# killerwhile/kafka-assignment-optimizer

Hardware: AMD Instinct MI355X
Metric: candidate assignments/sec (+ time_to_optimal_s), 10k-partition reassign (higher is better)
Workload: dtype int32

## Files before the change

### kafka_assignment_optimizer_amd/csrc/kao_search.hip

```cpp
#include "kao_search_dev.h"

namespace kao {

template <bool kGlobalA, bool kPriced, int NW, bool kWide, bool kTeam, bool kCurG = false, int RFT = 0>
__device__ __forceinline__ void search_body(unsigned char *smem, const SearchPools &pl, const SearchParams &prm) {
    static_assert(!kTeam || kGlobalA, "teams run topics that live in global memory");
    static_assert(!kCurG || !kGlobalA, "kCurG: the working assignment is in LDS");
    static_assert(RFT == 0 || (RFT == 3 && NW == 4 && !kGlobalA && !kTeam), "RFT = 3: LDS-resident topics of four words per partition");
    constexpr int NS = RFT ? RFT : NW;
    const int lane = threadIdx.x & 63;
    const int wave = __builtin_amdgcn_readfirstlane(threadIdx.x >> 6);
    const int n_waves = kTeam ? __builtin_amdgcn_readfirstlane((int)(blockDim.x >> 6)) : 1;
    const int tid = kTeam ? (int)threadIdx.x : lane, nthr = kTeam ? (int)blockDim.x : 64;
    const int2 bm = pl.block_map[blockIdx.x];
    const TopicDev *TD = pl.topics + bm.x;

    TopicRegs T = topic_regs<RFT>(TD);
    asm volatile("" : "+v"(T.rep_lo), "+v"(T.rep_hi), "+v"(T.lead_lo), "+v"(T.lead_hi));

    const int a_bytes = kGlobalA ? 0 : prm.maxP * NW * 4;
    const int cur_bytes = (kGlobalA || kCurG) ? 0 : prm.maxP * NW * 4;
    const int bx64 = (prm.maxBx + 63) & ~63;
    const int c_bytes = bx64 * 4;
    const int krt = search_rack_tab(prm.maxR);
// ... 164 lines not shown
    const uint32_t pmask = (1u << plog) - 1u;
    const uint32_t lrange = (uint32_t)(prm.lam_max - prm.lam_min + 1);
    const uint32_t RF8 = (uint32_t)T.RF << 8, R8 = (uint32_t)T.R << 8, m8 = (uint32_t)T.m << 8;

    const int T_tour = min(64, max(4, (T.P * T.RF) >> 2));
    uint32_t tour_off = lane < T_tour ? 0u : kKeyNull;
    asm volatile("" : "+v"(tour_off));
    const int GA = min(16, max(1, (T.P * T.RF) >> 8));
    const int x_rounds_full = (T.P + 63) >> 6;
    const bool x_windowed = x_rounds_full > 8;

    int lam_lo = prm.lam_min, lam_hi = prm.lam_max;
    uint32_t n_iters = prm.iters, it_base = prm.launch * prm.iters;
    uint32_t scan_two = TD->P * TD->RF <= prm.scan2_max ? 1u : 0u;
    {
        uint32_t v0 = (uint32_t)lam_lo, v1 = (uint32_t)lam_hi, v2 = n_iters, v3 = it_base, v4 = scan_two;
        asm volatile("" : "+v"(v0), "+v"(v1), "+v"(v2), "+v"(v3), "+v"(v4));
        lam_lo = (int)__builtin_amdgcn_readfirstlane(v0); lam_hi = (int)__builtin_amdgcn_readfirstlane(v1);
        n_iters = __builtin_amdgcn_readfirstlane(v2); it_base = __builtin_amdgcn_readfirstlane(v3);
        scan_two = __builtin_amdgcn_readfirstlane(v4);
    }
    constexpr bool kFuse = !kGlobalA && !kTeam && !kPriced;
    const bool fuse_ok = kFuse && T.Bx <= 16384;
    uint32_t jmp_a = 1u, jmp_c = 0u;
    if (fuse_ok)
        for (int n = (T.Bx + 63) >> 6; n > 0; --n) { jmp_a = (jmp_a * 0x6D2B79u) & 0xFFFFFFu; jmp_c = (jmp_c * 0x6D2B79u + 0x3C6EF3u) & 0xFFFFFFu; }
    for (uint32_t i = 0; i < n_iters; ++i) {
        const uint32_t it = it_base + i;
        const int type = (int)((0x1210u >> ((it & 7u) * 2u)) & 3u);
        const uint32_t ph = it & pmask;
        const int lam = best_obj < 0 ? lam_hi : min(lam_hi, lam_lo + (int)((2u * ph * lrange) >> plog));
        const bool sampled = (type == 2) || (type == 0 && ((it >> 3) & 1u));

        uint32_t key = kKeyNull;
        int dV = 0, dObj = 0, p = 0, k = 0, q = 0, j = 0;
        uint32_t uw = 0, vw = 0;
        uint32_t kmin;
        int win;

        if (sampled) {
            p = (int)rnd24_wide(rng, (uint32_t)T.P);
            const Part<NW> a = L.A[p];
            const Part<NW> c = CUR[p];
            if (type == 0) {
                k = (int)rnd24(rng, RF8);
                uw = sel_slot<NS>(a, k);
                const uint32_t ro = uw >> 16;
                const bool lead = k == 0;
                const uint32_t lw = lead ? 2u : 0u;
                const int wl = lead ? T.w00 : T.w01, wf = lead ? T.w10 : T.w11;
                const int g_old = role_w2<NS>(c, uw, wl, wf) + (hbw ? bw_of(BW[uw & 0xFFFFu], lead) : 0);
                const uint32_t wo = L.W[uw & 0xFFFFu];
                const int dV_old = wfld(wo, kWDecR) + wfldw(wo, kWDecL, lw);
                const int dV_rack_old = ddec(L.K[ro], T.rack_lo, T.rack_hi) + ddec(cnt4<NS>(a, ro), T.prack_lo, T.prack_hi);
                const int rsz_ro = RSZ[ro];
                int dP_old = 0, dP_rack_old = 0;
                if (kPriced) {
                    const uint32_t pro = PR[uw & 0xFFFFu];
                    dP_old = -(wflag(wo, kWPoutR) & price_rep(pro));
                    if (lead) dP_old -= wflag(wo, kWPoutL) & price_lead(pro);
                    dP_rack_old = p_out(L.K[ro], T.rack_lo, T.rack_hi, PG[ro]);
                }
#pragma unroll
                for (int g = 0; g < 4; ++g) {
                    uint32_t r, jj;
                    bool okg;
                    if (g < 2) {
                        r = rnd24(rng, R8);
                        jj = rnd24(rng, m8);
                        okg = (int)jj < RSZ[r];
                    } else {
                        r = ro;
                        jj = rnd24(rng, (uint32_t)rsz_ro << 8);
                        okg = true;
                    }
                    const uint32_t x = __umul24(r, (uint32_t)T.m) + jj;
                    const uint32_t xw = x | (r << 16);
                    okg = okg && !in4<NS>(a, xw);
                    const uint32_t wn = L.W[x];
                    int dVg = dV_old + wfld(wn, kWIncR) + wfldw(wn, kWIncL, lw);
                    if (g < 2) {
                        if (r != ro)
                            dVg += dV_rack_old + dinc(L.K[r], T.rack_lo, T.rack_hi) + dinc(cnt4<NS>(a, r), T.prack_lo, T.prack_hi);
                    }
                    const int dObjg = role_w2<NS>(c, xw, wl, wf) + (hbw ? bw_of(BW[x], lead) : 0) - g_old;
                    uint32_t keyg;
                    if (kPriced) {
                        const uint32_t prx = PR[x];
                        int dPg = dP_old + (wflag(wn, kWPinR) & price_rep(prx));
                        if (lead) dPg += wflag(wn, kWPinL) & price_lead(prx);
                        if (g < 2 && r != ro) dPg += dP_rack_old + p_in(L.K[r], T.rack_lo, T.rack_hi, PG[r]);
                        keyg = okg ? make_key_p(lam, S, dVg, dObjg, dPg, lane) : kKeyNull;
                    }
                    else keyg = okg ? make_key(lam, S, dVg, dObjg, lane) : kKeyNull;
                    if (keyg < key) { key = keyg; vw = xw; dV = dVg; dObj = dObjg; }
                }
            } else {
                uw = a.w[0];
                const int u_lead = role_w2<NS>(c, uw, T.w00, T.w10), u_fol = role_w2<NS>(c, uw, T.w01, T.w11);
                const uint32_t wu = L.W[uw & 0xFFFFu];
                const int dV_u = wfld(wu, kWDecL);
                const int dP_u = kPriced ? -(wflag(wu, kWPoutL) & price_lead(PR[uw & 0xFFFFu])) : 0;
#pragma unroll
                for (int kk = 1; kk < NS; ++kk) {
                    if (!RFT && kk >= T.RF) break;
                    const uint32_t xw = a.w[kk];
                    const int dObjg = role_w2<NS>(c, xw, T.w00, T.w10) + u_fol - u_lead - role_w2<NS>(c, xw, T.w01, T.w11) +
                                      (hbw ? (int)(BW[xw & 0xFFFFu] >> 16) - (int)(BW[uw & 0xFFFFu] >> 16) : 0);
                    const uint32_t wx = L.W[xw & 0xFFFFu];
                    const int dVg = dV_u + wfld(wx, kWIncL);
                    uint32_t keyg;
                    if (kPriced) keyg = make_key_p(lam, S, dVg, dObjg, dP_u + (wflag(wx, kWPinL) & price_lead(PR[xw & 0xFFFFu])), lane);
                    else keyg = make_key(lam, S, dVg, dObjg, lane);
                    if (keyg < key) { key = keyg; vw = xw; k = kk; dV = dVg; dObj = dObjg; }
                }
            }
            kmin = wave_umin(key);
            win = (int)(kmin & 63u);
        } else {
            uint32_t keyA, oldw_l;
            int pl_, kl_, g_old_l, dvo_l = 0, dvr_l = 0;
            auto score_words = [&](auto ty, uint32_t &key_o, const Part<NW> &al, const Part<NW> &cl, int k_o, uint32_t &oldw_o, int &g_o, int &dvo_o, int &dvr_o) {
                constexpr int TY = decltype(ty)::value;
                oldw_o = sel_slot<NS>(al, k_o);
                const uint32_t rol = oldw_o >> 16;
                const bool leadl = k_o == 0;
                g_o = role_w2<NS>(cl, oldw_o, leadl ? T.w00 : T.w01, leadl ? T.w10 : T.w11);
                if (hbw && TY == 0) g_o += bw_of(BW[oldw_o & 0xFFFFu], leadl);
                const uint32_t wo = L.W[oldw_o & 0xFFFFu];
                const int dv7 = ddec(cnt4<NS>(al, rol), T.prack_lo, T.prack_hi);
                int sc;
                if (TY == 0) {
                    dvo_o = wfld(wo, kWDecR) + wfldw(wo, kWDecL, leadl ? 2u : 0u);
                    dvr_o = ddec(L.K[rol], T.rack_lo, T.rack_hi) + dv7;
                    sc = dvo_o + min(dvr_o, 0);
                } else {
                    const int dvl = wfld(wo, leadl ? kWDecL : kWIncL);
                    sc = min(dv7, 0) + min(dvl, 0);
                }
                if (kPriced) {
                    int dPs = 0;
                    if (TY == 0) {
                        const uint32_t pro = PR[oldw_o & 0xFFFFu];
                        dPs = -(wflag(wo, kWPoutR) & price_rep(pro));
                        dPs -= wflagw(wo, kWPoutL, leadl ? 1u : 0u) & price_lead(pro);
                    }
                    key_o = make_key_p(lam, S, sc, -g_o, dPs, lane) | tour_off;
                }
                else key_o = make_key(lam, S, sc, -g_o, lane) | tour_off;
            };
            auto score_slot = [&](auto ty, uint32_t &key_o, int p_o, int &k_o, uint32_t &oldw_o, int &g_o, int &dvo_o, int &dvr_o) {
// ... 133 lines not shown
                    int d2 = __mul24(lam, inc + wfldw(w, kWIncL, lw2) + (rt >> 16)) + K02;
                    if (decltype(with_w)::value) {
                        const uint32_t x = (uint32_t)(base + lane);
                        const uint32_t xw = x | ((uint32_t)XR[x] << 16);
                        d1 -= __mul24(S, role_w2<NS>(c1, xw, wl1, wf1));
                        d2 -= __mul24(S, role_w2<NS>(c2, xw, wl2, wf2));
                    }
                    d1 = min(max(d1, 0), 2 * kDBias - 2);
                    d2 = min(max(d2, 0), 2 * kDBias - 2) | wflag(w, 14);
                    key1 = ((uint32_t)d1 << 16) | (st1 & 0xFF00u) | (uint32_t)rd | ((uint32_t)w & 0xFFFF0000u);
                    key2 = ((uint32_t)d2 << 16) | (st2 & 0xFF00u) | (uint32_t)rd;
                };
                const int n_rd = (T.Bx + 63) >> 6;
                int rd = 0, base = 0;
                while (rd < n_rd) {
                    int nxt = n_rd;
#pragma unroll
                    for (int i2 = 0; i2 < 2 * NW; ++i2)
                        if (mr[i2] >= rd) nxt = min(nxt, mr[i2]);
                    uint32_t k1a, k2a, k1b, k2b;
                    for (; rd + 1 < nxt; rd += 2, base += 128) {
                        scan_round2(std::false_type{}, base, rd, k1a, k2a);
                        scan_round2(std::false_type{}, base + 64, rd + 1, k1b, k2b);
                        best1 = min(best1, min(k1a, k1b));
                        best2 = min(best2, min(k2a, k2b));
                    }
                    if (rd < nxt) { scan_round2(std::false_type{}, base, rd, k1a, k2a); best1 = min(best1, k1a); best2 = min(best2, k2a); ++rd; base += 64; }
                    if (rd < n_rd) { scan_round2(std::true_type{}, base, rd, k1a, k2a); best1 = min(best1, k1a); best2 = min(best2, k2a); ++rd; base += 64; }
                }
                asm("v_mad_u32_u24 %0, %0, %1, %2" : "+v"(rng) : "s"(jmp_a), "v"(jc));
                if (holds) L.W[ai & 0xFFFFu] = (uint16_t)w_keep;
                const uint32_t kw = wave_umin(min(((best1 >> 1) & ~127u) | (uint32_t)lane, ((best2 >> 1) & ~127u) | 64u | (uint32_t)lane));
                const bool two = (kw & 64u) != 0u;
                kmin = kw >> 7;
                win = (int)(kw & 63u);
                p = two ? ps[1] : ps[0]; k = two ? ks[1] : ks[0]; uw = two ? us[1] : us[0];
                if ((int)(kmin >> 8) - kDBias <= 0) {
                    const bool lead = k == 0;
                    const uint32_t bw_ = (uint32_t)__builtin_amdgcn_readlane((int)(two ? best2 : best1), win);
                    const uint32_t xs = ((bw_ & 255u) << 6) + (uint32_t)win;
                    const uint32_t rs = XR[xs];
                    const uint32_t ws = L.W[xs];
                    const int rts = L.RT[rs];
                    vw = xs | (rs << 16);
                    dV = wfld(ws, kWIncR) + wfldw(ws, kWIncL, lead ? 2u : 0u) + (two ? dvos[1] : dvos[0]) + (two ? (rts >> 16) : wfldw(rts, 0, 16u));
                    int mx1 = -1, mx2 = -1;
#pragma unroll
                    for (int i2 = 0; i2 < NW; ++i2) { mx1 = max(mx1, mr[i2]); mx2 = max(mx2, mr[NW + i2]); }
                    const bool has_missing = (two ? mx2 : mx1) >= 0;
                    dObj = -(two ? gs[1] : gs[0]) + (has_missing ? (two ? role_w2<NS>(c2, vw, wl2, wf2) : role_w2<NS>(c1, vw, wl1, wf1)) : 0);
                }
            } else {
            uint32_t b_kmin = kKeyNull, b_uw = 0, b_vw = 0;
            int b_win = 0, b_p = 0, b_k = 0, b_dV = 0, b_dObj = 0;
#pragma nounroll
            for (int si = 0; si < (wA2 >= 0 ? 2 : 1); ++si) {
            const int wA = si == 0 ? wA1 : wA2;
            p = __builtin_amdgcn_readlane(pl_, wA);
            k = __builtin_amdgcn_readlane(kl_, wA);
            uw = (uint32_t)__builtin_amdgcn_readlane((int)oldw_l, wA);
            const int g_old = __builtin_amdgcn_readlane(g_old_l, wA);
            const int dV_old = __builtin_amdgcn_readlane(dvo_l, wA);
            const int dV_rack_old = __builtin_amdgcn_readlane(dvr_l, wA);
            Part<NW> a, c;
            if constexpr (kGlobalA) {
#pragma unroll
                for (int i2 = 0; i2 < NW; ++i2) { a.w[i2] = (uint32_t)__builtin_amdgcn_readlane((int)a_l.w[i2], wA); c.w[i2] = (uint32_t)__builtin_amdgcn_readlane((int)c_l.w[i2], wA); }
            } else {
                a = L.A[p];
                c = CUR[p];
            }
            const bool lead = k == 0;
            const uint32_t ro = uw >> 16;
            if (type == 0) {
                {
                    const int dP_rack_old = kPriced ? p_out(L.K[ro], T.rack_lo, T.rack_hi, PG[ro]) : 0;
                    for (int r = lane; r < T.R; r += 64) {
                        int v = ((uint32_t)r != ro) ? dV_rack_old + dinc(L.K[r], T.rack_lo, T.rack_hi) + dinc(cnt4<NS>(a, (uint32_t)r), T.prack_lo, T.prack_hi) : 0;
                        if (kPriced)
                            v = (v & 0xFF) | ((((uint32_t)r != ro) ? dP_rack_old + p_in(L.K[r], T.rack_lo, T.rack_hi, PG[r]) : 0) * 256);
                        L.RT[r] = v;
                    }
                }
                const int wl = lead ? T.w00 : T.w01, wf = lead ? T.w10 : T.w11;
                const int li = lane & (NW - 1);
                const uint32_t ai = sel_slot<NS>(a, li), ci = sel_slot<NS>(c, li);
                const bool holds = (lane < NS) & (ai != kNoneW);
                uint32_t w_keep = 0;
                if (!kTeam && holds) {
                    w_keep = L.W[ai & 0xFFFFu];
                    L.W[ai & 0xFFFFu] = (uint16_t)(w_keep | kWNoCand);
                }
                int ar[NS];
                {
                    const int ar_l = (kTeam && holds) ? (int)((ai & 0xFFFFu) >> 6) : -1;
#pragma unroll
                    for (int i2 = 0; i2 < NS; ++i2) ar[i2] = __builtin_amdgcn_readlane(ar_l, i2);
                }
                const bool hm_l = (lane < NS) & (ci != kNoneW) & !in4<NS>(a, ci);
                const int mr_l = hm_l ? (int)((ci & 0xFFFFu) >> 6) : -1;
                int mr[NS];
#pragma unroll
                for (int i2 = 0; i2 < NS; ++i2) mr[i2] = __builtin_amdgcn_readlane(mr_l, i2);
                bool has_missing = false;
#pragma unroll
                for (int i2 = 0; i2 < NS; ++i2) has_missing |= mr[i2] >= 0;
                int K0 = __mul24(S, g_old) + kDBias + __mul24(lam, dV_old);
// ... 47 lines not shown
                                bestc = min(bestc, is_weighted(rdg) ? scan_round(std::true_type{}, base, rd) : scan_round(std::false_type{}, base, rd));
                                bestc = min(bestc, is_weighted(rdg + 1) ? scan_round(std::true_type{}, base + 64, rd + 1) : scan_round(std::false_type{}, base + 64, rd + 1));
                            } else {
                                const uint32_t k0 = scan_round(std::false_type{}, base, rd);
                                const uint32_t k1 = scan_round(std::false_type{}, base + 64, rd + 1);
                                bestc = min(bestc, min(k0, k1));
                            }
                        }
                    }
                    if (kWide || kTeam) {
                        for (; base < cend; base += 64, ++rd)
                            bestc = min(bestc, is_weighted((cb >> 6) + rd) ? scan_round(std::true_type{}, base, rd) : scan_round(std::false_type{}, base, rd));
                    } else {
                        const int n_rd = (cend - cb + 63) >> 6, rd0 = cb >> 6;
                        while (rd < n_rd) {
                            int nxt = n_rd;
#pragma unroll
                            for (int i2 = 0; i2 < NS; ++i2) {
                                const int m = mr[i2] - rd0;
                                if (m >= rd) nxt = min(nxt, m);
                            }
                            for (; rd + 1 < nxt; rd += 2, base += 128) {
                                const uint32_t k0 = scan_round(std::false_type{}, base, rd);
                                const uint32_t k1 = scan_round(std::false_type{}, base + 64, rd + 1);
                                bestc = min(bestc, min(k0, k1));
                            }
                            if (rd < nxt) { bestc = min(bestc, scan_round(std::false_type{}, base, rd)); ++rd; base += 64; }
                            if (rd < n_rd) { bestc = min(bestc, scan_round(std::true_type{}, base, rd)); ++rd; base += 64; }
                        }
                    }
                    if ((bestc >> 8) < (bestA >> 8)) { bestA = bestc; chunkA = cb; }
                }
                if (!kTeam && holds) L.W[ai & 0xFFFFu] = (uint16_t)w_keep;
                key = bestA >> 8;
                kmin = wave_umin(key);
                const unsigned long long bal = __ballot(key == kmin);
                win = __ffsll((long long)bal) - 1;
                if ((int)(kmin >> 8) - kDBias <= 0) {
                    const uint32_t bw_ = (uint32_t)__builtin_amdgcn_readlane((int)bestA, win);
                    const uint32_t xs = (uint32_t)__builtin_amdgcn_readlane(chunkA, win) + ((bw_ & 255u) << 6) + (uint32_t)win;
                    const uint32_t rs = XR[xs];
                    const uint32_t ws = L.W[xs];
                    const int rts = L.RT[rs];
                    vw = xs | (rs << 16);
                    dV = wfld(ws, kWIncR) + wfldw(ws, kWIncL, lw) + dV_old + (kPriced ? (int)(signed char)(rts & 0xFF) : rts);
                    dObj = -g_old + (has_missing ? role_w2<NS>(c, vw, wl, wf) : 0) + (hbw ? bw_of(BW[xs], lead) : 0);
                }
                if (si == 0 || kmin < b_kmin) { b_kmin = kmin; b_win = win; b_p = p; b_k = k; b_uw = uw; b_vw = vw; b_dV = dV; b_dObj = dObj; }
            } else {
                const int nrp = lead ? 0 : 1;
                const int cnt_a_ru = cnt4<NS>(a, ro);
                const uint32_t wu = L.W[uw & 0xFFFFu];
                const int pl_u = kPriced ? price_lead(PR[uw & 0xFFFFu]) : 0;
                const int bwl_u = hbw ? (int)(BW[uw & 0xFFFFu] >> 16) : 0;
                if (!kGlobalA) {
                    const int q_draw = (int)rnd24_wide(rng, (uint32_t)T.P);
                    q0 = x_windowed ? __builtin_amdgcn_readfirstlane(q_draw) : 0;
                }
                const int x_rounds = x_windowed ? 8 : x_rounds_full;
                auto x_round = [&](int rd, const Part<NW> &b, const Part<NW> &cb) {
                    const uint32_t tie0 = lcg24(rng) >> 8;
                    int qq; bool okq;
                    x_partner(rd, qq, okq);
                    okq = okq & (qq != p);
                    const bool u_in_b = in4<NS>(b, uw);
                    const int u_in_q_lead = role_w2<NS>(cb, uw, T.w00, T.w10), u_in_q_fol = role_w2<NS>(cb, uw, T.w01, T.w11);
                    const int dv_ro = ddec(cnt_a_ru, T.prack_lo, T.prack_hi) + dinc(cnt4<NS>(b, ro), T.prack_lo, T.prack_hi);
                    int cnt_b_rv[3] = {0, 0, 0};
                    if constexpr (RFT == 3) {
                        const int e01 = (int)((b.w[0] >> 16) == (b.w[1] >> 16)), e02 = (int)((b.w[0] >> 16) == (b.w[2] >> 16)), e12 = (int)((b.w[1] >> 16) == (b.w[2] >> 16));
                        cnt_b_rv[0] = 1 + e01 + e02; cnt_b_rv[1] = 1 + e01 + e12; cnt_b_rv[2] = 1 + e02 + e12;
                    }
#pragma unroll
                    for (int jj = 0; jj < NS; ++jj) {
                        if (!RFT && jj >= T.RF) break;
                        const uint32_t v = b.w[jj];
                        const bool ok = okq & (v != uw) & !in4<NS>(a, v) & !u_in_b;
                        const int nrq = jj != 0;
                        int dObjx = role_w<NS>(T, c, v, nrp) + (jj == 0 ? u_in_q_lead : u_in_q_fol) - g_old - role_w<NS>(T, cb, v, nrq);
                        int dVx = 0, dPx = 0;
                        if (lead != (jj == 0)) {
                            const uint32_t wv = L.W[v & 0xFFFFu];
// ... 5 lines not shown
                                           : ((wflag(wu, kWPinL) & pl_u) - (wflag(wv, kWPoutL) & plv));
                            }
                        }
                        const uint32_t rv = v >> 16;
                        if (rv != ro)
                            dVx += dv_ro + dinc(cnt4<NS>(a, rv), T.prack_lo, T.prack_hi) + ddec(RFT == 3 ? cnt_b_rv[jj < 3 ? jj : 0] : cnt4<NS>(b, rv), T.prack_lo, T.prack_hi);
                        uint32_t keyx;
                        if (kPriced) keyx = ok ? make_key_tie_p(lam, S, dVx, dObjx, dPx, tie0 + (uint32_t)jj * 0x55u) : kKeyNull;
                        else keyx = ok ? make_key_tie(lam, S, dVx, dObjx, tie0 + (uint32_t)jj * 0x55u) : kKeyNull;
                        if (keyx < key) { key = keyx; vw = v; q = qq; j = jj; dV = dVx; dObj = dObjx; }
                    }
                };
                if constexpr (kGlobalA) {
#pragma unroll
                    for (int r2 = 0; r2 < XB; ++r2)
                        if (r2 < x_rounds) x_round(r2, xb[r2], xcb[r2]);
                    for (int rb = XB; rb < x_rounds; rb += XB) {
                        Part<NW> yb[XB], ycb[XB];
#pragma unroll
                        for (int r2 = 0; r2 < XB; ++r2) { int qq; bool okq; const int qc = x_partner(rb + r2, qq, okq); yb[r2] = L.A[qc]; ycb[r2] = CUR[qc]; }
#pragma unroll
                        for (int r2 = 0; r2 < XB; ++r2)
                            if (rb + r2 < x_rounds) x_round(rb + r2, yb[r2], ycb[r2]);
                    }
                } else {
                    for (int rd = 0; rd < x_rounds; ++rd) {
                        int qq; bool okq;
                        const int qc = x_partner(rd, qq, okq);
                        const Part<NW> b = L.A[qc];
                        const Part<NW> cb = CUR[qc];
                        x_round(rd, b, cb);
                    }
                }
                kmin = wave_umin(key);
                const unsigned long long bal = __ballot(key == kmin);
                win = __ffsll((long long)bal) - 1;
            }
            }
            if (type == 0) { kmin = b_kmin; win = b_win; p = b_p; k = b_k; uw = b_uw; vw = b_vw; dV = b_dV; dObj = b_dObj; }
            }
        }
        if (!kTeam) {
            if (kmin == kKeyNull) continue;
            if ((int)(kmin >> 8) - kDBias > 0) continue;
        }
        bool mine = true;
        int *rec = TR + ((i & 1u) * 16 + (uint32_t)wave) * kTeamRec;
        if (kTeam) {
            const bool ok = kmin != kKeyNull && (int)(kmin >> 8) - kDBias <= 0;
            if (lane == win) {
                const uint32_t ro_ = uw >> 16, rn_ = vw >> 16;
                const bool racks = ok && type == 0 && ro_ != rn_;
                rec[0] = ok ? 1 : 0; rec[1] = p; rec[2] = type == 1 ? q : p;
                rec[3] = (int)(uw & 0xFFFFu); rec[4] = (int)(vw & 0xFFFFu);
                rec[5] = racks ? (int)ro_ : 0xFFFF; rec[6] = racks ? (int)rn_ : 0xFFFF;
                rec[7] = dV; rec[8] = dObj;
            }
            __syncthreads();
            bool clash = false;
            if (lane < wave) {
                const int *o = TR + ((i & 1u) * 16 + (uint32_t)lane) * kTeamRec;
                if (o[0]) {
                    const int mp = rec[1], mq = rec[2], mb0 = rec[3], mb1 = rec[4], mr0 = rec[5], mr1 = rec[6];
                    clash = (o[1] == mp) | (o[1] == mq) | (o[2] == mp) | (o[2] == mq) | (o[3] == mb0) | (o[3] == mb1) | (o[4] == mb0) | (o[4] == mb1);
                    if (o[5] != 0xFFFF && mr0 != 0xFFFF) clash |= (o[5] == mr0) | (o[5] == mr1) | (o[6] == mr0) | (o[6] == mr1);
                }
            }
            mine = ok && __ballot(clash) == 0ull;
        }

        if (lane == win && mine) {
            uint32_t *ap = reinterpret_cast<uint32_t *>(&L.A[p]);
            if (type == 0) {
                const uint32_t d = (k == 0) ? 0x10001u : 1u;
                L.C[uw & 0xFFFFu] -= d;
                L.C[vw & 0xFFFFu] += d;
                if (!kTeam || (uw >> 16) != (vw >> 16)) {
                    L.K[uw >> 16] -= 1;
                    L.K[vw >> 16] += 1;
                }
                ap[k] = vw;
            } else if (type == 1) {
                uint32_t *bp = reinterpret_cast<uint32_t *>(&L.A[q]);
                if ((k == 0) != (j == 0)) {
                    const uint32_t lose = (k == 0) ? uw : vw, gain = (k == 0) ? vw : uw;
                    L.C[lose & 0xFFFFu] -= 0x10000u;
                    L.C[gain & 0xFFFFu] += 0x10000u;
                }
                ap[k] = vw;
                bp[j] = uw;
            } else {
                L.C[uw & 0xFFFFu] -= 0x10000u;
                L.C[vw & 0xFFFFu] += 0x10000u;
                ap[0] = vw;
                ap[k] = uw;
            }
        }
        if (mine) {
            const int k_lead = __builtin_amdgcn_readlane(k, win) == 0 ? 2 : 0;
            int rows;
            if (type == 0) rows = 1 | k_lead;
            else if (type == 1) rows = k_lead ^ (__builtin_amdgcn_readlane(j, win) == 0 ? 2 : 0);
            else rows = 2;
            if (rows != 0) {
                const uint32_t xo = (uint32_t)__builtin_amdgcn_readlane((int)uw, win) & 0xFFFFu, xn = (uint32_t)__builtin_amdgcn_readlane((int)vw, win) & 0xFFFFu;
                uint32_t xx = xo;
                asm("v_writelane_b32 %0, %1, 1" : "+v"(xx) : "s"(xn));
                int lane_w = lane;
                asm volatile("" : "+v"(lane_w));
                if (lane_w < 2) {
                    const uint32_t cx = L.C[xx];
                    uint32_t wx;
                    if (rows == 3) wx = band_fields(T, cx);
                    else if (rows == 1) wx = (L.W[xx] & ~kWRowR) | band_entry((int)(cx & 0xFFFFu), T.rep_lo, T.rep_hi);
                    else wx = (L.W[xx] & ~kWRowL) | (band_entry((int)(cx >> 16), T.lead_lo, T.lead_hi) << 6);
                    L.W[xx] = (uint16_t)wx;
                }
            }
        }
        if (kGlobalA) __builtin_amdgcn_fence(__ATOMIC_SEQ_CST, "workgroup");
        if (kTeam) {
            if (lane == 0) rec[9] = mine ? 1 : 0;
            __syncthreads();
            int dVs = 0, dOs = 0, na = 0;
            if (lane < n_waves) {
                const int *o = TR + ((i & 1u) * 16 + (uint32_t)lane) * kTeamRec;
                if (o[9]) { dVs = o[7]; dOs = o[8]; na = 1; }
            }
            V += wave_sum(dVs);
            obj += wave_sum(dOs);
            accepted += wave_sum(na);
        } else {
            V += __builtin_amdgcn_readlane(dV, win);
            obj += __builtin_amdgcn_readlane(dObj, win);
            accepted++;
        }
        if (V == 0 && obj > best_obj) { best_obj = obj; snapshot(T, L, ext, best, tid, nthr); }
    }

    if (kTeam) __syncthreads();
    recount(T, L, tid, nthr, krt);
    if (kTeam) __syncthreads();
    int V2, obj2;
    full_cost<NW, kTeam>(T, L, CUR, RSZ, tid, nthr, V2, obj2, hbw ? BW : nullptr, TS, wave, n_waves);
    if ((V2 != V || obj2 != obj) && tid == 0) atomicAdd(pl.drift, 1);
    if (!kGlobalA)
        for (int p = lane; p < T.P; p += 64) store_packed<NW>(state_packed, p, L.A[p]);
    if (tid == 0) {
        pl.restart_info[g * 4 + 0] = best_obj;
        pl.restart_info[g * 4 + 1] = V2;
        pl.restart_info[g * 4 + 2] = obj2;
        pl.restart_info[g * 4 + 3] = accepted;
    }
}

#ifndef KAO_WPE_SMALL
#define KAO_WPE_SMALL 6
#endif
#ifndef KAO_WPE_WIDE
#define KAO_WPE_WIDE 6
#endif
template <bool kGlobalA, bool kPriced, int NW, bool kWide> constexpr int search_min_waves() { return kGlobalA ? 1 : (kWide ? KAO_WPE_WIDE : KAO_WPE_SMALL); }
template <bool kGlobalA, bool kPriced, int NW, bool kWide, int RFT = 0>
__global__ __launch_bounds__(256) __attribute__((amdgpu_waves_per_eu(search_min_waves<kGlobalA, kPriced, NW, kWide>(), 8))) void k_search(SearchPools pl, SearchParams prm) {
    extern __shared__ __attribute__((aligned(16))) unsigned char smem[];
    search_body<kGlobalA, kPriced, NW, kWide, false, false, RFT>(smem, pl, prm);
}
template <bool kPriced, int NW>
// ... 217 lines not shown
```

### kafka_assignment_optimizer_amd/csrc/kao_search_dev.h

```cpp
#pragma once
#include <hip/hip_runtime.h>

#include <type_traits>

#include "kao_device.h"
#include "kao_internal.h"

namespace kao {

__device__ __forceinline__ uint32_t fmix32(uint32_t h) {
    h ^= h >> 16; h *= 0x85EBCA6Bu; h ^= h >> 13; h *= 0xC2B2AE35u; h ^= h >> 16;
    return h;
}
__device__ __forceinline__ uint32_t xs32(uint32_t &s) {
    s ^= s << 13; s ^= s >> 17; s ^= s << 5;
    return s;
}
__device__ __forceinline__ uint32_t mulhi(uint32_t a, uint32_t b) { return __umulhi(a, b); }
__device__ __forceinline__ int band(int c, int lo, int hi) { return max(c - hi, 0) + max(lo - c, 0); }
__device__ __forceinline__ int dinc(int c, int lo, int hi) { return (int)(c >= hi) - (int)(c < lo); }
__device__ __forceinline__ int ddec(int c, int lo, int hi) { return (int)(c <= lo) - (int)(c > hi); }

template <int NW> struct alignas(16) Part { uint32_t w[NW]; };
__device__ __forceinline__ uint32_t sel4(const Part<4> &a, int k) {
// ... 21 lines not shown
__device__ __forceinline__ uint32_t rnd24_wide(uint32_t &s, uint32_t n) {
    const uint32_t v = lcg24(s);
    return __umulhi((v & 0xFFFFFFu) << 8, n);
}
__device__ __forceinline__ uint32_t key_of(int delta, uint32_t low) {
    delta = min(max(delta, -kDBias), kDBias - 2);
    return ((uint32_t)(delta + kDBias) << 8) | low;
}
__device__ __forceinline__ uint32_t make_key_p(int lam, int S, int dV, int dObj, int dP, int lane) { return key_of(__mul24(lam, dV) - __mul24(S, dObj) + dP, (uint32_t)lane); }
__device__ __forceinline__ uint32_t make_key(int lam, int S, int dV, int dObj, int lane) { return key_of(__mul24(lam, dV) - __mul24(S, dObj), (uint32_t)lane); }
__device__ __forceinline__ uint32_t make_key_tie_p(int lam, int S, int dV, int dObj, int dP, uint32_t tie) { return key_of(__mul24(lam, dV) - __mul24(S, dObj) + dP, tie & 0xFFu); }
__device__ __forceinline__ uint32_t make_key_tie(int lam, int S, int dV, int dObj, uint32_t tie) { return key_of(__mul24(lam, dV) - __mul24(S, dObj), tie & 0xFFu); }
__device__ __forceinline__ int price_rep(uint32_t pr) { return (int)(short)(pr & 0xFFFFu); }
__device__ __forceinline__ int price_lead(uint32_t pr) { return (int)pr >> 16; }
__device__ __forceinline__ int p_in(int c, int lo, int hi, int price) { return ((c >= hi) | (c < lo)) ? price : 0; }
__device__ __forceinline__ int p_out(int c, int lo, int hi, int price) { return ((c > hi) | (c <= lo)) ? -price : 0; }
__device__ __forceinline__ int bw_of(uint32_t bw, bool lead) { return (int)(bw & 0xFFFFu) + (lead ? (int)(bw >> 16) : 0); }
__device__ __forceinline__ int price_units(int v, int S) { return min(max((S * v + kDualScale / 2) >> kDualLog2, -32767), 32767); }

template <int NS = 0, int NW> __device__ __forceinline__ bool in4(const Part<NW> &a, uint32_t w) {
    bool r = false;
#pragma unroll
    for (int i = 0; i < (NS ? NS : NW); ++i) r |= a.w[i] == w;
    return r;
}
template <int NS = 0, int NW> __device__ __forceinline__ int cnt4(const Part<NW> &a, uint32_t r) {
    int n = 0;
#pragma unroll
    for (int i = 0; i < (NS ? NS : NW); ++i) n += (int)((a.w[i] >> 16) == r);
    return n;
}
template <int NS, int NW> __device__ __forceinline__ uint32_t sel_slot(const Part<NW> &a, int k) {
    if constexpr (NS == 3 && NW == 4) {
        uint32_t w0 = a.w[0], w1 = a.w[1], w2 = a.w[2];
        asm("" : "+v"(w0), "+v"(w1), "+v"(w2));
        return (k & 2) ? w2 : ((k & 1) ? w1 : w0);
    } else return sel4(a, k);
}

struct TopicRegs {
    int P, RF, R, m, Bx;
    uint32_t magic;
    int rep_lo, rep_hi, lead_lo, lead_hi, rack_lo, rack_hi, prack_lo, prack_hi;
    int w00, w01, w10, w11;
};

template <int RFT = 0> __device__ __forceinline__ TopicRegs topic_regs(const TopicDev *TD) {
    TopicRegs T;
    T.P = TD->P; T.RF = RFT ? RFT : TD->RF; T.R = TD->R; T.m = TD->m; T.Bx = TD->Bx; T.magic = TD->magic;
    T.rep_lo = TD->rep_lo; T.rep_hi = TD->rep_hi; T.lead_lo = TD->lead_lo; T.lead_hi = TD->lead_hi;
    T.rack_lo = TD->rack_lo; T.rack_hi = TD->rack_hi; T.prack_lo = TD->prack_lo; T.prack_hi = TD->prack_hi;
    T.w00 = TD->w00; T.w01 = TD->w01; T.w10 = TD->w10; T.w11 = TD->w11;
    return T;
}

template <int NS = 0, int NW> __device__ __forceinline__ int role_w2(const Part<NW> &c, uint32_t w, int wl, int wf) {
    bool fol = false;
#pragma unroll
    for (int i = 1; i < (NS ? NS : NW); ++i) fol |= c.w[i] == w;
    return (c.w[0] == w) ? wl : (fol ? wf : 0);
}
template <int NS = 0, int NW> __device__ __forceinline__ int role_w(const TopicRegs &T, const Part<NW> &c, uint32_t w, int nr) {
    return role_w2<NS>(c, w, nr ? T.w01 : T.w00, nr ? T.w11 : T.w10);
}
__device__ __forceinline__ uint32_t to_word(const TopicRegs &T, uint32_t x) {
    return x == 0xFFFFu ? kNoneW : (x | (mulhi(x, T.magic) << 16));
}
template <int NW> __device__ __forceinline__ Part<NW> load_packed(const TopicRegs &T, const unsigned char *base, int p) {
    Part<NW> a;
// ... 133 lines not shown
```

Baseline: 773.2 billion.

## Specialize move commit per move type via templated finish lambda

Moves the shared accept/commit tail of the search loop into a lambda, templated on move type and on whether the move fields are already wave-uniform. Each branch calls it directly, so the runtime type checks and the readlanes of already-uniform values can be resolved at compile time. Variables that were shared across branches become branch-local, which may ease register pressure. Also changes how sel_slot hides values from the optimizer, so the slot index rather than the words is opaque. The cost is code duplication from instantiating the tail several times, which could raise instruction-cache pressure.

```diff
diff --git a/kafka_assignment_optimizer_amd/csrc/kao_search.hip b/kafka_assignment_optimizer_amd/csrc/kao_search.hip
--- a/kafka_assignment_optimizer_amd/csrc/kao_search.hip
+++ b/kafka_assignment_optimizer_amd/csrc/kao_search.hip
@@ -220,19 +220,117 @@
         const int lam = best_obj < 0 ? lam_hi : min(lam_hi, lam_lo + (int)((2u * ph * lrange) >> plog));
         const bool sampled = (type == 2) || (type == 0 && ((it >> 3) & 1u));
 
-        uint32_t key = kKeyNull;
-        int dV = 0, dObj = 0, p = 0, k = 0, q = 0, j = 0;
-        uint32_t uw = 0, vw = 0;
-        uint32_t kmin;
-        int win;
+        auto finish = [&](auto ty, auto uni, uint32_t kmin, int win, int p, int k, int q, int j, uint32_t uw, uint32_t vw, int dV, int dObj) {
+            constexpr int TY = decltype(ty)::value;
+            auto of_win = [&](int v) { return decltype(uni)::value ? v : __builtin_amdgcn_readlane(v, win); };
+            if (!kTeam) {
+                if (kmin == kKeyNull) return;
+                if ((int)(kmin >> 8) - kDBias > 0) return;
+            }
+            bool mine = true;
+            int *rec = TR + ((i & 1u) * 16 + (uint32_t)wave) * kTeamRec;
+            if (kTeam) {
+                const bool ok = kmin != kKeyNull && (int)(kmin >> 8) - kDBias <= 0;
+                if (lane == win) {
+                    const uint32_t ro_ = uw >> 16, rn_ = vw >> 16;
+                    const bool racks = ok && TY == 0 && ro_ != rn_;
+                    rec[0] = ok ? 1 : 0; rec[1] = p; rec[2] = TY == 1 ? q : p;
+                    rec[3] = (int)(uw & 0xFFFFu); rec[4] = (int)(vw & 0xFFFFu);
+                    rec[5] = racks ? (int)ro_ : 0xFFFF; rec[6] = racks ? (int)rn_ : 0xFFFF;
+                    rec[7] = dV; rec[8] = dObj;
+                }
+                __syncthreads();
+                bool clash = false;
+                if (lane < wave) {
+                    const int *o = TR + ((i & 1u) * 16 + (uint32_t)lane) * kTeamRec;
+                    if (o[0]) {
+                        const int mp = rec[1], mq = rec[2], mb0 = rec[3], mb1 = rec[4], mr0 = rec[5], mr1 = rec[6];
+                        clash = (o[1] == mp) | (o[1] == mq) | (o[2] == mp) | (o[2] == mq) | (o[3] == mb0) | (o[3] == mb1) | (o[4] == mb0) | (o[4] == mb1);
+                        if (o[5] != 0xFFFF && mr0 != 0xFFFF) clash |= (o[5] == mr0) | (o[5] == mr1) | (o[6] == mr0) | (o[6] == mr1);
+                    }
+                }
+                mine = ok && __ballot(clash) == 0ull;
+            }
+
+            if (lane == win && mine) {
+                uint32_t *ap = reinterpret_cast<uint32_t *>(&L.A[p]);
+                if (TY == 0) {
+                    const uint32_t d = (k == 0) ? 0x10001u : 1u;
+                    L.C[uw & 0xFFFFu] -= d;
+                    L.C[vw & 0xFFFFu] += d;
+                    if (!kTeam || (uw >> 16) != (vw >> 16)) {
+                        L.K[uw >> 16] -= 1;
+                        L.K[vw >> 16] += 1;
+                    }
+                    ap[k] = vw;
+                } else if (TY == 1) {
+                    uint32_t *bp = reinterpret_cast<uint32_t *>(&L.A[q]);
+                    if ((k == 0) != (j == 0)) {
+                        const uint32_t lose = (k == 0) ? uw : vw, gain = (k == 0) ? vw : uw;
+                        L.C[lose & 0xFFFFu] -= 0x10000u;
+                        L.C[gain & 0xFFFFu] += 0x10000u;
+                    }
+                    ap[k] = vw;
+                    bp[j] = uw;
+                } else {
+                    L.C[uw & 0xFFFFu] -= 0x10000u;
+                    L.C[vw & 0xFFFFu] += 0x10000u;
+                    ap[0] = vw;
+                    ap[k] = uw;
+                }
+            }
+            if (mine) {
+                int rows;
+                if (TY == 0) rows = 1 | (of_win(k) == 0 ? 2 : 0);
+                else if (TY == 1) rows = (of_win(k) == 0 ? 2 : 0) ^ (of_win(j) == 0 ? 2 : 0);
+                else rows = 2;
+                if (rows != 0) {
+                    const uint32_t xo = (uint32_t)of_win((int)uw) & 0xFFFFu, xn = decltype(uni)::value ? (uint32_t)__builtin_amdgcn_readfirstlane((int)(vw & 0xFFFFu)) : (uint32_t)of_win((int)vw) & 0xFFFFu;
+                    uint32_t xx = xo;
+                    asm("v_writelane_b32 %0, %1, 1" : "+v"(xx) : "s"(xn));
+                    int lane_w = lane;
+                    asm volatile("" : "+v"(lane_w));
+                    if (lane_w < 2) {
+                        const uint32_t cx = L.C[xx];
+                        uint32_t wx;
+                        if (rows == 3) wx = band_fields(T, cx);
+                        else if (rows == 1) wx = (L.W[xx] & ~kWRowR) | band_entry((int)(cx & 0xFFFFu), T.rep_lo, T.rep_hi);
+                        else wx = (L.W[xx] & ~kWRowL) | (band_entry((int)(cx >> 16), T.lead_lo, T.lead_hi) << 6);
+                        L.W[xx] = (uint16_t)wx;
+                    }
+                }
+            }
+            if (kGlobalA) __builtin_amdgcn_fence(__ATOMIC_SEQ_CST, "workgroup");
+            if (kTeam) {
+                if (lane == 0) rec[9] = mine ? 1 : 0;
+                __syncthreads();
+                int dVs = 0, dOs = 0, na = 0;
+                if (lane < n_waves) {
+                    const int *o = TR + ((i & 1u) * 16 + (uint32_t)lane) * kTeamRec;
+                    if (o[9]) { dVs = o[7]; dOs = o[8]; na = 1; }
+                }
+                V += wave_sum(dVs);
+                obj += wave_sum(dOs);
+                accepted += wave_sum(na);
+            } else {
+                V += of_win(dV);
+                obj += of_win(dObj);
+                accepted++;
+            }
+        };
+        constexpr std::integral_constant<int, 0> kReplace{};
+        constexpr std::integral_constant<int, 1> kExchange{};
+        constexpr std::integral_constant<int, 2> kLeaderSwap{};
 
         if (sampled) {
-            p = (int)rnd24_wide(rng, (uint32_t)T.P);
+            const int p = (int)rnd24_wide(rng, (uint32_t)T.P);
             const Part<NW> a = L.A[p];
             const Part<NW> c = CUR[p];
+            uint32_t key = kKeyNull, vw = 0;
+            int dV = 0, dObj = 0;
             if (type == 0) {
-                k = (int)rnd24(rng, RF8);
-                uw = sel_slot<NS>(a, k);
+                const int k = (int)rnd24(rng, RF8);
+                const uint32_t uw = sel_slot<NS>(a, k);
                 const uint32_t ro = uw >> 16;
                 const bool lead = k == 0;
                 const uint32_t lw = lead ? 2u : 0u;
@@ -283,8 +381,11 @@
                     else keyg = okg ? make_key(lam, S, dVg, dObjg, lane) : kKeyNull;
                     if (keyg < key) { key = keyg; vw = xw; dV = dVg; dObj = dObjg; }
                 }
+                const uint32_t kmin = wave_umin(key);
+                finish(kReplace, std::false_type{}, kmin, (int)(kmin & 63u), p, k, 0, 0, uw, vw, dV, dObj);
             } else {
-                uw = a.w[0];
+                const uint32_t uw = a.w[0];
+                int k = 0;
                 const int u_lead = role_w2<NS>(c, uw, T.w00, T.w10), u_fol = role_w2<NS>(c, uw, T.w01, T.w11);
                 const uint32_t wu = L.W[uw & 0xFFFFu];
                 const int dV_u = wfld(wu, kWDecL);
@@ -302,9 +403,9 @@
                     else keyg = make_key(lam, S, dVg, dObjg, lane);
                     if (keyg < key) { key = keyg; vw = xw; k = kk; dV = dVg; dObj = dObjg; }
                 }
-            }
-            kmin = wave_umin(key);
-            win = (int)(kmin & 63u);
+                const uint32_t kmin = wave_umin(key);
+                finish(kLeaderSwap, std::false_type{}, kmin, (int)(kmin & 63u), p, k, 0, 0, uw, vw, dV, dObj);
+            }
         } else {
             uint32_t keyA, oldw_l;
             int pl_, kl_, g_old_l, dvo_l = 0, dvr_l = 0;
@@ -504,9 +605,10 @@
                 if (holds) L.W[ai & 0xFFFFu] = (uint16_t)w_keep;
                 const uint32_t kw = wave_umin(min(((best1 >> 1) & ~127u) | (uint32_t)lane, ((best2 >> 1) & ~127u) | 64u | (uint32_t)lane));
                 const bool two = (kw & 64u) != 0u;
-                kmin = kw >> 7;
-                win = (int)(kw & 63u);
-                p = two ? ps[1] : ps[0]; k = two ? ks[1] : ks[0]; uw = two ? us[1] : us[0];
+                const uint32_t kmin = kw >> 7;
+                const int win = (int)(kw & 63u);
+                const int p = two ? ps[1] : ps[0], k = two ? ks[1] : ks[0];
+                const uint32_t uw = two ? us[1] : us[0];
                 if ((int)(kmin >> 8) - kDBias <= 0) {
                     const bool lead = k == 0;
                     const uint32_t bw_ = (uint32_t)__builtin_amdgcn_readlane((int)(two ? best2 : best1), win);
@@ -514,37 +616,44 @@
                     const uint32_t rs = XR[xs];
                     const uint32_t ws = L.W[xs];
                     const int rts = L.RT[rs];
-                    vw = xs | (rs << 16);
-                    dV = wfld(ws, kWIncR) + wfldw(ws, kWIncL, lead ? 2u : 0u) + (two ? dvos[1] : dvos[0]) + (two ? (rts >> 16) : wfldw(rts, 0, 16u));
+                    const uint32_t vw = xs | (rs << 16);
+                    const int dV = wfld(ws, kWIncR) + wfldw(ws, kWIncL, lead ? 2u : 0u) + (two ? dvos[1] : dvos[0]) + (two ? (rts >> 16) : wfldw(rts, 0, 16u));
                     int mx1 = -1, mx2 = -1;
 #pragma unroll
                     for (int i2 = 0; i2 < NW; ++i2) { mx1 = max(mx1, mr[i2]); mx2 = max(mx2, mr[NW + i2]); }
                     const bool has_missing = (two ? mx2 : mx1) >= 0;
-                    dObj = -(two ? gs[1] : gs[0]) + (has_missing ? (two ? role_w2<NS>(c2, vw, wl2, wf2) : role_w2<NS>(c1, vw, wl1, wf1)) : 0);
+                    const int dObj = -(two ? gs[1] : gs[0]) + (has_missing ? (two ? role_w2<NS>(c2, vw, wl2, wf2) : role_w2<NS>(c1, vw, wl1, wf1)) : 0);
+                    finish(kReplace, std::true_type{}, kmin, win, p, k, 0, 0, uw, vw, dV, dObj);
                 }
             } else {
+            auto slot_of = [&](int wA, int &p, int &k, uint32_t &uw, int &g_old, int &dV_old, int &dV_rack_old, Part<NW> &a, Part<NW> &c) {
+                p = __builtin_amdgcn_readlane(pl_, wA);
+                k = __builtin_amdgcn_readlane(kl_, wA);
+                uw = (uint32_t)__builtin_amdgcn_readlane((int)oldw_l, wA);
+                g_old = __builtin_amdgcn_readlane(g_old_l, wA);
+                dV_old = __builtin_amdgcn_readlane(dvo_l, wA);
+                dV_rack_old = __builtin_amdgcn_readlane(dvr_l, wA);
+                if constexpr (kGlobalA) {
+#pragma unroll
+                    for (int i2 = 0; i2 < NW; ++i2) { a.w[i2] = (uint32_t)__builtin_amdgcn_readlane((int)a_l.w[i2], wA); c.w[i2] = (uint32_t)__builtin_amdgcn_readlane((int)c_l.w[i2], wA); }
+                } else {
+                    a = L.A[p];
+                    c = CUR[p];
+                }
+            };
+            if (type == 0) {
             uint32_t b_kmin = kKeyNull, b_uw = 0, b_vw = 0;
             int b_win = 0, b_p = 0, b_k = 0, b_dV = 0, b_dObj = 0;
 #pragma nounroll
             for (int si = 0; si < (wA2 >= 0 ? 2 : 1); ++si) {
-            const int wA = si == 0 ? wA1 : wA2;
-            p = __builtin_amdgcn_readlane(pl_, wA);
-            k = __builtin_amdgcn_readlane(kl_, wA);
-            uw = (uint32_t)__builtin_amdgcn_readlane((int)oldw_l, wA);
-            const int g_old = __builtin_amdgcn_readlane(g_old_l, wA);
-            const int dV_old = __builtin_amdgcn_readlane(dvo_l, wA);
-            const int dV_rack_old = __builtin_amdgcn_readlane(dvr_l, wA);
-            Part<NW> a, c;
-            if constexpr (kGlobalA) {
-#pragma unroll
-                for (int i2 = 0; i2 < NW; ++i2) { a.w[i2] = (uint32_t)__builtin_amdgcn_readlane((int)a_l.w[i2], wA); c.w[i2] = (uint32_t)__builtin_amdgcn_readlane((int)c_l.w[i2], wA); }
-            } else {
-                a = L.A[p];
-                c = CUR[p];
-            }
-            const bool lead = k == 0;
-            const uint32_t ro = uw >> 16;
-            if (type == 0) {
+                int p, k, g_old, dV_old, dV_rack_old;
+                uint32_t uw;
+                Part<NW> a, c;
+                slot_of(si == 0 ? wA1 : wA2, p, k, uw, g_old, dV_old, dV_rack_old, a, c);
+                const bool lead = k == 0;
+                const uint32_t ro = uw >> 16;
+                uint32_t vw = 0;
+                int dV = 0, dObj = 0;
                 {
                     const int dP_rack_old = kPriced ? p_out(L.K[ro], T.rack_lo, T.rack_hi, PG[ro]) : 0;
                     for (int r = lane; r < T.R; r += 64) {
@@ -658,10 +767,10 @@
                     if ((bestc >> 8) < (bestA >> 8)) { bestA = bestc; chunkA = cb; }
                 }
                 if (!kTeam && holds) L.W[ai & 0xFFFFu] = (uint16_t)w_keep;
-                key = bestA >> 8;
-                kmin = wave_umin(key);
+                const uint32_t key = bestA >> 8;
+                const uint32_t kmin = wave_umin(key);
                 const unsigned long long bal = __ballot(key == kmin);
-                win = __ffsll((long long)bal) - 1;
+                const int win = __ffsll((long long)bal) - 1;
                 if ((int)(kmin >> 8) - kDBias <= 0) {
                     const uint32_t bw_ = (uint32_t)__builtin_amdgcn_readlane((int)bestA, win);
                     const uint32_t xs = (uint32_t)__builtin_amdgcn_readlane(chunkA, win) + ((bw_ & 255u) << 6) + (uint32_t)win;
@@ -673,7 +782,17 @@
                     dObj = -g_old + (has_missing ? role_w2<NS>(c, vw, wl, wf) : 0) + (hbw ? bw_of(BW[xs], lead) : 0);
                 }
                 if (si == 0 || kmin < b_kmin) { b_kmin = kmin; b_win = win; b_p = p; b_k = k; b_uw = uw; b_vw = vw; b_dV = dV; b_dObj = dObj; }
+            }
+            finish(kReplace, std::true_type{}, b_kmin, b_win, b_p, b_k, 0, 0, b_uw, b_vw, b_dV, b_dObj);
             } else {
+                int p, k, g_old, dV_old, dV_rack_old;
+                uint32_t uw;
+                Part<NW> a, c;
+                slot_of(wA1, p, k, uw, g_old, dV_old, dV_rack_old, a, c);
+                const bool lead = k == 0;
+                const uint32_t ro = uw >> 16;
+                uint32_t key = kKeyNull, vw = 0;
+                int dV = 0, dObj = 0, q = 0, j = 0;
                 const int nrp = lead ? 0 : 1;
                 const int cnt_a_ru = cnt4<NS>(a, ro);
                 const uint32_t wu = L.W[uw & 0xFFFFu];
@@ -745,108 +864,12 @@
                         x_round(rd, b, cb);
                     }
                 }
-                kmin = wave_umin(key);
+                const uint32_t kmin = wave_umin(key);
                 const unsigned long long bal = __ballot(key == kmin);
-                win = __ffsll((long long)bal) - 1;
-            }
-            }
-            if (type == 0) { kmin = b_kmin; win = b_win; p = b_p; k = b_k; uw = b_uw; vw = b_vw; dV = b_dV; dObj = b_dObj; }
-            }
-        }
-        if (!kTeam) {
-            if (kmin == kKeyNull) continue;
-            if ((int)(kmin >> 8) - kDBias > 0) continue;
-        }
-        bool mine = true;
-        int *rec = TR + ((i & 1u) * 16 + (uint32_t)wave) * kTeamRec;
-        if (kTeam) {
-            const bool ok = kmin != kKeyNull && (int)(kmin >> 8) - kDBias <= 0;
-            if (lane == win) {
-                const uint32_t ro_ = uw >> 16, rn_ = vw >> 16;
-                const bool racks = ok && type == 0 && ro_ != rn_;
-                rec[0] = ok ? 1 : 0; rec[1] = p; rec[2] = type == 1 ? q : p;
-                rec[3] = (int)(uw & 0xFFFFu); rec[4] = (int)(vw & 0xFFFFu);
-                rec[5] = racks ? (int)ro_ : 0xFFFF; rec[6] = racks ? (int)rn_ : 0xFFFF;
-                rec[7] = dV; rec[8] = dObj;
-            }
-            __syncthreads();
-            bool clash = false;
-            if (lane < wave) {
-                const int *o = TR + ((i & 1u) * 16 + (uint32_t)lane) * kTeamRec;
-                if (o[0]) {
-                    const int mp = rec[1], mq = rec[2], mb0 = rec[3], mb1 = rec[4], mr0 = rec[5], mr1 = rec[6];
-                    clash = (o[1] == mp) | (o[1] == mq) | (o[2] == mp) | (o[2] == mq) | (o[3] == mb0) | (o[3] == mb1) | (o[4] == mb0) | (o[4] == mb1);
-                    if (o[5] != 0xFFFF && mr0 != 0xFFFF) clash |= (o[5] == mr0) | (o[5] == mr1) | (o[6] == mr0) | (o[6] == mr1);
-                }
-            }
-            mine = ok && __ballot(clash) == 0ull;
-        }
-
-        if (lane == win && mine) {
-            uint32_t *ap = reinterpret_cast<uint32_t *>(&L.A[p]);
-            if (type == 0) {
-                const uint32_t d = (k == 0) ? 0x10001u : 1u;
-                L.C[uw & 0xFFFFu] -= d;
-                L.C[vw & 0xFFFFu] += d;
-                if (!kTeam || (uw >> 16) != (vw >> 16)) {
-                    L.K[uw >> 16] -= 1;
-                    L.K[vw >> 16] += 1;
-                }
-                ap[k] = vw;
-            } else if (type == 1) {
-                uint32_t *bp = reinterpret_cast<uint32_t *>(&L.A[q]);
-                if ((k == 0) != (j == 0)) {
-                    const uint32_t lose = (k == 0) ? uw : vw, gain = (k == 0) ? vw : uw;
-                    L.C[lose & 0xFFFFu] -= 0x10000u;
-                    L.C[gain & 0xFFFFu] += 0x10000u;
-                }
-                ap[k] = vw;
-                bp[j] = uw;
-            } else {
-                L.C[uw & 0xFFFFu] -= 0x10000u;
-                L.C[vw & 0xFFFFu] += 0x10000u;
-                ap[0] = vw;
-                ap[k] = uw;
-            }
-        }
-        if (mine) {
-            const int k_lead = __builtin_amdgcn_readlane(k, win) == 0 ? 2 : 0;
-            int rows;
-            if (type == 0) rows = 1 | k_lead;
-            else if (type == 1) rows = k_lead ^ (__builtin_amdgcn_readlane(j, win) == 0 ? 2 : 0);
-            else rows = 2;
-            if (rows != 0) {
-                const uint32_t xo = (uint32_t)__builtin_amdgcn_readlane((int)uw, win) & 0xFFFFu, xn = (uint32_t)__builtin_amdgcn_readlane((int)vw, win) & 0xFFFFu;
-                uint32_t xx = xo;
-                asm("v_writelane_b32 %0, %1, 1" : "+v"(xx) : "s"(xn));
-                int lane_w = lane;
-                asm volatile("" : "+v"(lane_w));
-                if (lane_w < 2) {
-                    const uint32_t cx = L.C[xx];
-                    uint32_t wx;
-                    if (rows == 3) wx = band_fields(T, cx);
-                    else if (rows == 1) wx = (L.W[xx] & ~kWRowR) | band_entry((int)(cx & 0xFFFFu), T.rep_lo, T.rep_hi);
-                    else wx = (L.W[xx] & ~kWRowL) | (band_entry((int)(cx >> 16), T.lead_lo, T.lead_hi) << 6);
-                    L.W[xx] = (uint16_t)wx;
-                }
-            }
-        }
-        if (kGlobalA) __builtin_amdgcn_fence(__ATOMIC_SEQ_CST, "workgroup");
-        if (kTeam) {
-            if (lane == 0) rec[9] = mine ? 1 : 0;
-            __syncthreads();
-            int dVs = 0, dOs = 0, na = 0;
-            if (lane < n_waves) {
-                const int *o = TR + ((i & 1u) * 16 + (uint32_t)lane) * kTeamRec;
-                if (o[9]) { dVs = o[7]; dOs = o[8]; na = 1; }
-            }
-            V += wave_sum(dVs);
-            obj += wave_sum(dOs);
-            accepted += wave_sum(na);
-        } else {
-            V += __builtin_amdgcn_readlane(dV, win);
-            obj += __builtin_amdgcn_readlane(dObj, win);
-            accepted++;
+                const int win = __ffsll((long long)bal) - 1;
+                finish(kExchange, std::false_type{}, kmin, win, p, k, q, j, uw, vw, dV, dObj);
+            }
+            }
         }
         if (V == 0 && obj > best_obj) { best_obj = obj; snapshot(T, L, ext, best, tid, nthr); }
     }
diff --git a/kafka_assignment_optimizer_amd/csrc/kao_search_dev.h b/kafka_assignment_optimizer_amd/csrc/kao_search_dev.h
--- a/kafka_assignment_optimizer_amd/csrc/kao_search_dev.h
+++ b/kafka_assignment_optimizer_amd/csrc/kao_search_dev.h
@@ -77,9 +77,10 @@
 }
 template <int NS, int NW> __device__ __forceinline__ uint32_t sel_slot(const Part<NW> &a, int k) {
     if constexpr (NS == 3 && NW == 4) {
-        uint32_t w0 = a.w[0], w1 = a.w[1], w2 = a.w[2];
-        asm("" : "+v"(w0), "+v"(w1), "+v"(w2));
-        return (k & 2) ? w2 : ((k & 1) ? w1 : w0);
+        int k1 = k & 1, k2 = k & 2;
+        asm("" : "+v"(k1), "+v"(k2));
+        const uint32_t w0 = a.w[0], w1 = a.w[1], w2 = a.w[2];
+        return k2 ? w2 : (k1 ? w1 : w0);
     } else return sel4(a, k);
 }
 
```

After: 822.2 billion, median of 6. 1.06x the previous value.
